# MarcoMeter/endless-memory-gym

Hardware: AMD Instinct MI355X
Metric: env steps/sec (aggregate) (higher is better)
Workload: dtype u8; 1 GPU; MortarMayhem-Grid-v0, 65536 envs/GPU x 1 GPU, 84x84x3 obs (u8_xyc), same-step auto-reset, uniform random actions generated on device; env_id=MortarMayhem-Grid-v0, envs_per_gpu=65536, envs_total=65536, parallelism=env-sharded x1, no data-path collective

## Files before the change

endless-memory-gym_amd/csrc/mg_mortar.hip:

```cpp
#include <memory>

#include "mg_atlas_v1.hpp"
#include "mg_lab.hpp"
#include "mg_option_sets.hpp"
#include "mg_stamps.hpp"
#include "mg_mortar_types.hpp"
#include "mg_mortar_compose.hpp"
#include "mg_mortar_step.hpp"
#include "mg_mortar_one_launch.hpp"

namespace mg {
using namespace v1;

__global__ __launch_bounds__(256) void mortar_init_kernel(int n, MortarState* state) {
    int i = blockIdx.x * blockDim.x + threadIdx.x;
    if (i >= n) return;
    MortarState s;
    memset(&s, 0, sizeof(s));
    s.disp_sprite = 0xFF;
    state[i] = s;
}

__global__ __launch_bounds__(256) void mortar_gt64_kernel(int n, const MortarState* state, double* out) {
    const int i = blockIdx.x * blockDim.x + threadIdx.x;
    if (i >= n) return;
    const MortarState s = state[i];
    out[2 * i] = s.tx / 5.0;
    out[2 * i + 1] = s.ty / 5.0;
}

__global__ __launch_bounds__(256) void mortar_debug_desc_kernel(MortarParams P0, int n, MortarIO io, MortarDesc* out) {
    const int i = blockIdx.x * blockDim.x + threadIdx.x;
    if (i >= n) return;
    const MortarParams& P = io.set_of ? io.sets[set_index(io.set_of, i)] : P0;
    const MortarState s = io.state[i];
    const uint8_t* cmds = io.cmds + (size_t)i * P.cmd_cap;
    MortarDesc d = io.desc[i];
    {
        const bool have = s.disp_sprite != 0xFF;
        const int cx = (have && !s.disp_is_agent) ? s.disp_x : s.ax, cy = (have && !s.disp_is_agent) ? s.disp_y : s.ay;
        d.sx = (int16_t)(cx - P.sprite_dim / 2);
        d.sy = (int16_t)(cy - P.sprite_dim / 2);
        d.sprite = have ? s.disp_sprite : (uint8_t)0;
        d.tmpl = (uint16_t)((s.tiles_on && P.visual_feedback) ? 1 + s.tx * P.N + s.ty : 0);
        d.glyph_x0 = (int16_t)P.glyph_x0;
    }
    d.glyph = 0xFF;
    if (s.vis_pos < s.vis_len) {
        const int idx = (int)s.dbg_pops, period = s.show_dur + s.show_delay;
        io.state[i].dbg_pops = s.dbg_pops + 1;
        if (idx >= 0 && idx < (int)s.vis_len && period > 0) {
            const int k = idx / period, w = idx % period;
            d.glyph = (w < s.show_dur) ? cmds[s.vis_base + k] : (uint8_t)9;
        }
    }
    const int r = P.tile / 2;
    d.ring_x = (int16_t)(P.arena_x0 + P.tile * s.tx + P.tile / 2 - r);
    d.ring_y = (int16_t)(P.arena_x0 + P.tile * s.ty + P.tile / 2 - r);
    d.ring_on = 1;
    out[i] = d;
}

static const double SCALE = 0.25;

class MortarFamily : public Family {
   public:
    MortarFamily(int variant_id, int n) : Family(n), P_(sets_[0].P) {
        memset(&P_, 0, sizeof(P_));
        const int variant = variant_id >= 3 ? variant_id - 3 : variant_id;
        P_.variant = variant;
        P_.taskb = variant_id >= 3;
        agent_scale_ = 1.0 * SCALE;
        agent_speed_ = 12.0 * SCALE;
        P_.N = variant == V_ENDLESS ? 6 : 5;
        P_.allowed = variant == V_GRID ? 5 : 9;
        P_.visual_feedback = 1;
        P_.max_steps = -1;
        P_.initial_count = 1;
        P_.cmd_cap = variant == V_ENDLESS ? 512 : 32;
        if (variant == V_ENDLESS) {
            const int cap = lab_int("MEMGYM_EMM_CMD_CAP", 0);
            if (cap >= 4 && cap <= 512) P_.cmd_cap = cap;
        }
        MortarOpt& O = sets_[0];
        O.st_command_count.set(P_.command_count, {10});
        O.st_show_dur.set(P_.show_dur, {3});
        O.st_show_delay.set(P_.show_delay, {1});
        O.st_expl_dur.set(P_.expl_dur, {variant == V_GRID ? 2 : 6});
        O.st_expl_delay.set(P_.expl_delay, {variant == V_GRID ? 6 : 18});
        P_.r_fail = 0.0;
        P_.r_succ = 0.1;
        P_.r_ep_succ = 0.0;
        P_.r_new = 0.0;
        state_.alloc(n);
        cmds_.alloc((size_t)n * P_.cmd_cap);
        desc_.alloc(n);
        tdesc_.alloc(n);
        rng_.alloc(n);
        err_.alloc();
        claims_.alloc((size_t)((n + 255) / 256) * 4);
        rescues_.alloc(1);
        sets_.alloc();
        launch(mortar_init_kernel, dim3((n + 255) / 256), dim3(256), 0, 0, n, state_.p);
        MG_HIP(hipDeviceSynchronize());
        rebuild();
        sets_.defaults = P_;
    }

    void set_capacity(const std::string& what, int64_t v) override {
        if (!(P_.variant == V_ENDLESS && what == "commands")) return Family::set_capacity(what, v);
        if (v < 4 || v > 32768) throw OptionError{-3, "commands: 4 .. 32,768"};
        if (seeded_) throw std::runtime_error("mg_set_capacity: before the first reset");
        if (2 * P_.initial_count > v) throw OptionError{-3, "commands: below twice the initial_command_count in force"};
        MG_HIP(hipDeviceSynchronize());
        P_.cmd_cap = (int)v;
        cmds_.alloc((size_t)n_ * P_.cmd_cap);
        sets_.refresh_geometry();
    }
    int64_t capacity(const std::string& what) const override {
        if (P_.variant == V_ENDLESS && what == "commands") return P_.cmd_cap;
        return Family::capacity(what);
    }
    void want_done_flag(uint32_t* flag_dev, uint32_t ticket) override {
        flag_dev_ = flag_dev;
        flag_ticket_ = ticket;
    }
    bool done_flag_stored() override {
        const bool stored = flag_stored_;
        flag_stored_ = false;
        return stored;
    }
    int action_dim() const override { return P_.variant == V_GRID ? 1 : 2; }
    int gt_dim() const override { return P_.variant == V_ENDLESS ? 2 : 0; }
    int vec_dim() const override { return P_.taskb ? VEC_DIM : 0; }
    void bind_vector_obs(float* dev) override { vec_ = dev; }
    const char* info_name(int k) const override {
        if (P_.variant == V_ENDLESS) return k == 0 ? "commands_completed" : (k == 1 ? "max_command_sequence" : nullptr);
        return k == 0 ? "success" : (k == 1 ? "commands_completed" : nullptr);
    }

    void set_option(const std::string& key, const double* v, int n) override { set_option_set(0, key, v, n); }
    void set_option_set(int set, const std::string& key, const double* v, int n) override {
        MortarOpt& O = sets_.ensure(set);
        MortarParams& P = O.P;
        const bool endless = P_.variant == V_ENDLESS;
        const OptionArg A{set, key, v, n, dirty_};
        if (key == "agent_scale") A.geometry(agent_scale_, v[0]);
        else if (key == "allowed_commands") {
            int a = A.integer();
            if (a < 4 || a > 9) throw OptionError{-4, "assert 4 <= allowed_commands <= 9"};
            P.allowed = a;
        }
        else if (!P_.taskb && key == "command_show_duration") O.st_show_dur.set(P.show_dur, A.int_list(1, 65535));
        else if (!P_.taskb && key == "command_show_delay") O.st_show_delay.set(P.show_delay, A.int_list(0, 65535));
        else if (key == "explosion_duration") O.st_expl_dur.set(P.expl_dur, A.int_list(1, 65535));
        else if (key == "explosion_delay") O.st_expl_delay.set(P.expl_delay, A.int_list(1, 65535));
        else if (key == "visual_feedback") P.visual_feedback = A.flag();
        else if (key == "reward_command_failure") P.r_fail = v[0];
        else if (key == "reward_command_success") P.r_succ = v[0];
        else if (endless && key == "max_steps") P.max_steps = A.integer();
        else if (endless && key == "initial_command_count") {
            int c = A.integer();
            if (c < 1 || c > P_.cmd_cap / 2) throw OptionError{-3, "initial_command_count out of the supported range"};
            P.initial_count = c;
        }
        else if (endless && key == "reward_new_command_success") P.r_new = v[0];
        else if (!endless && key == "arena_size") {
            int a = A.integer();
            if (a < 2 || a > 6) throw OptionError{-4, "assert 2 <= arena_size <= 6"};
            if (a != P_.N) A.geometry(P_.N, a);
        }
        else if (!endless && key == "command_count") O.st_command_count.set(P.command_count, A.int_list(1, P_.taskb ? VEC_DIM / 9 : P_.cmd_cap));
        else if (!endless && key == "reward_episode_success") P.r_ep_succ = v[0];
        else if (P_.variant != V_GRID && key == "agent_speed") A.geometry(agent_speed_, v[0]);
        else throw OptionError{-2, "unknown reset parameter " + key};
    }
    void bind_option_sets(const int32_t* set_of_dev) override { sets_.bind(set_of_dev); }

    void reset(const int64_t* seeds, const uint8_t* mask, void* obs, float* gt, hipStream_t s) override {
        if (dirty_) rebuild();
        require_seeded(seeds);
        for (size_t k = 0; k < sets_.size(); ++k) {
            const MortarOpt& O = sets_[k];
            const long long n_max = P_.variant == V_ENDLESS ? O.P.initial_count : O.st_command_count.max(O.P.command_count);
            if (!P_.taskb && n_max * ((long long)O.st_show_dur.max(O.P.show_dur) + O.st_show_delay.max(O.P.show_delay)) > 65535)
                throw OptionError{-3, "command_count x (command_show_duration + command_show_delay) exceeds the 65,535 entries of this build's display schedule"};
        }
        if (seeds) seeded_ = true;
        sets_.upload(s);
        with_bool(sets_.per_set(), [&](auto PS) {
            launch(mortar_reset_kernel<decltype(PS)::value>, dim3((n_ + 255) / 256), dim3(256), 0, s, P_, n_, io(), seeds, mask, gt_dim() ? gt : nullptr);
        });
        reset_frames(mask, [&](const uint8_t* m) { launch_raster_sparse<MortarComposer>(desc_.p, atlas_->dev(), obs, obs_format, n_, s, m); },
                     [&] { raster(obs, s); });
    }

    void step(const int32_t* actions, void* obs, float* reward, uint8_t* done, float* gt, const mg_info_buffers* info,
              int autoreset, hipStream_t s) override {
        struct Consume {
            uint32_t*& flag;
            ~Consume() { flag = nullptr; }
        } consume{flag_dev_};
        flag_stored_ = false;
        const mg_info_buffers ib = begin_step(info);
        sets_.upload(s);
        const MortarStepArgs sa{P_, n_, io(), actions, reward, done, gt_dim() ? gt : nullptr, ib, autoreset, nullptr};
        if (one_byte_format() && fuse_step() && !sets_.per_set() && !capturing(s)) {
            epoch_ = epoch_ % 255u + 1u;
            ++ticket_;
            const int logic_wgs = (n_ + 255) / 256;
            const int frames = frames_grid(n_);
            static const bool logic_last = lab_flag("MEMGYM_LAB_LOGIC_LAST", false);
            const bool store_flag = flag_dev_ && n_ == 1 && gt_dim() == 0 && obs_format == MG_OBS_U8_XYC;
            auto one_launch = [&](auto kernel, const MortarStepArgs& a, uint32_t* flag, uint32_t flag_ticket) {
                launch(kernel, dim3(logic_wgs + frames), dim3(256), RASTER_LDS, s, a, logic_wgs, logic_last ? frames : 0, epoch_, ticket_,
                               claims_.p, rescues_.p, atlas_->dev(), obs, flag, flag_ticket);
            };
            prof.begin(1, s);
            if (store_flag) {
                one_launch(mortar_step_raster_kernel<true>, sa, flag_dev_, flag_ticket_);
            } else if (ib.final_obs_dev && autoreset) {
                MortarStepArgs fa = sa;
                fa.tdesc = tdesc_.p;
                with_one_byte_format(obs_format, [&](auto F) { one_launch(mortar_step_raster_kernel<false, true, decltype(F)::value>, fa, nullptr, 0u); });
            } else {
                with_one_byte_format(obs_format, [&](auto F) { one_launch(mortar_step_raster_kernel<false, false, decltype(F)::value>, sa, nullptr, 0u); });
            }
            check_launch();
            ++one_launch_steps_;
            flag_stored_ = store_flag;
            prof.end(1, s);
            return;
        }
        prof.begin(0, s);
        const int sb = step_block(256);
        with_bool(sets_.per_set(), [&](auto PS) { launch(mortar_step_kernel<decltype(PS)::value>, dim3((n_ + sb - 1) / sb), dim3(sb), 0, s, sa); });
        end_logic(s);
        prof.begin(1, s);
        raster(obs, s);
        prof.end(1, s);
    }

    std::vector<std::pair<void*, size_t>> state_blobs() override {
        std::vector<std::pair<void*, size_t>> v = {{state_.p, state_.bytes()}, {cmds_.p, cmds_.bytes()}};
        rng_.blobs(v);
        return v;
    }

    void ground_truth64(double* out, hipStream_t s) override {
        if (!gt_dim() || !out) return;
        launch_checked(mortar_gt64_kernel, dim3((n_ + 255) / 256), dim3(256), 0, s, n_, state_.p, out);
    }
    bool debug_counter(const std::string& name, int64_t* out) override {
        if (name == "cmd_list_max" || name == "cmd_list_ge12") {
            std::vector<MortarState> h(n_);
            MG_HIP(hipDeviceSynchronize());
            MG_HIP(hipMemcpy(h.data(), state_.p, sizeof(MortarState) * (size_t)n_, hipMemcpyDeviceToHost));
            int64_t mx = 0, ge = 0;
            for (const MortarState& s : h) {
                mx = s.num_cmds > mx ? s.num_cmds : mx;
                ge += s.num_cmds >= 12;
            }
            *out = name == "cmd_list_max" ? mx : ge;
            return true;
        }
        if (name == "one_launch_steps") {
            *out = one_launch_steps_;
            return true;
        }
        if (name != "one_launch_rescues") return false;
        uint32_t v = 0;
        MG_HIP(hipMemcpy(&v, rescues_.p, sizeof v, hipMemcpyDeviceToHost));
        *out = (int64_t)v;
        return true;
    }

    void raster_debug(void* frames, hipStream_t s) override {
        debug_frames<MortarDesc>(
            s, [&](MortarDesc* dbg) { launch(mortar_debug_desc_kernel, dim3((n_ + 255) / 256), dim3(256), 0, s, P_, n_, io(), dbg); },
            [&](MortarDesc* dbg) { launch_raster<MortarDebugComposer>(dbg, atlas_->dev(), frames, MG_OBS_U8_XYC, n_, s); });
    }

   private:
    uint32_t* flag_dev_ = nullptr;
    uint32_t flag_ticket_ = 0;
    bool flag_stored_ = false;
    int64_t one_launch_steps_ = 0;
    uint32_t ticket_ = 0;
    uint32_t epoch_ = 0;
    bool one_byte_format() const { return obs_format == MG_OBS_U8_XYC || obs_format == MG_OBS_U8_CYX; }
    static bool fuse_step() {
        static const bool on = lab_flag("MEMGYM_MORTAR_FUSE", true);
        return on;
    }
    static bool capturing(hipStream_t s) {
        hipStreamCaptureStatus st = hipStreamCaptureStatusNone;
        return hipStreamIsCapturing(s, &st) == hipSuccess && st != hipStreamCaptureStatusNone;
    }
    MortarIO io() {
        MortarIO o;
        o.state = state_.p;
        o.cmds = cmds_.p;
        o.rng = rng_.view();
        o.desc = desc_.p;
        o.vec = vec_;
        o.err = err_.dev;
        o.sets = sets_.dev();
        o.set_of = sets_.set_of();
        return o;
    }

    void rebuild() {
        int radius = 0;
        std::vector<Stamp> sprites = build_agent_sprites(P_.variant == V_GRID ? 1.0 * SCALE : agent_scale_, &radius);
        std::vector<Stamp> glyphs = build_glyphs(SCALE);
        P_.tile = (int)(56 * SCALE);
        P_.arena_x0 = SCREEN / 2 - ((P_.tile * P_.N) >> 1);
        P_.radius = radius;
        P_.sprite_dim = sprites[0].w;
        double inv = 1.0 / std::sqrt(2.0);
        P_.v_axis = (1.0 / 1.0) * agent_speed_;
        P_.v_diag = inv * agent_speed_;
        P_.v_axis_i = (int)P_.v_axis;
        P_.v_diag_i = (int)P_.v_diag;
        P_.off_lo = (int)(-8 * SCALE);
        P_.off_hi = (int)(8 * SCALE);

        atlas_.reset(new Atlas());
        for (auto& sp : sprites) atlas_->add_stamp(sp);
        for (auto& g : glyphs) atlas_->add_stamp(g);
        {
            const int r = P_.tile / 2;
            Stamp ring_stamp(2 * r, 2 * r);
            circle(ring_stamp, r, r, r, (int)(8 * SCALE), 6);
            atlas_->add_stamp(ring_stamp);
        }
        atlas_->set_templates(build_mortar_templates(P_.N, SCALE, SCREEN));
        atlas_->upload();
        P_.glyph_x0 = (int)((SCREEN / 2) - std::floor(88 * SCALE / 2));
        dirty_ = false;
        sets_.refresh_geometry();
    }

    struct MortarOpt {
        MortarParams P;
        OptListStore st_command_count, st_show_dur, st_show_delay, st_expl_dur, st_expl_delay;
        static void copy_geometry(MortarParams& d, const MortarParams& s) {
            d.variant = s.variant; d.N = s.N; d.taskb = s.taskb; d.cmd_cap = s.cmd_cap; d.arena_x0 = s.arena_x0; d.tile = s.tile;
            d.radius = s.radius; d.sprite_dim = s.sprite_dim; d.glyph_x0 = s.glyph_x0; d.v_axis_i = s.v_axis_i; d.v_diag_i = s.v_diag_i;
            d.off_lo = s.off_lo; d.off_hi = s.off_hi; d.v_axis = s.v_axis; d.v_diag = s.v_diag;
        }
    };

    void raster_only(void* obs, const uint8_t* only, hipStream_t s) override {
        launch_raster<MortarComposer>(desc_.p, atlas_->dev(), obs, obs_format, n_, s, only);
        check_launch();
    }
    bool keeps_final_obs(hipStream_t s) override {
        static const bool wanted = lab_flag("MEMGYM_MORTAR_FINAL_FUSED", true);
        return wanted && one_byte_format() && fuse_step() && !sets_.per_set() && !capturing(s);
    }

    void raster(void* obs, hipStream_t s) { raster_only(obs, nullptr, s); }

    OptionSets<MortarOpt> sets_;
    MortarParams& P_;
    std::unique_ptr<Atlas> atlas_;
    double agent_scale_, agent_speed_;
    float* vec_ = nullptr;
    DevArray<MortarState> state_;
    DevArray<uint8_t> cmds_;
    DevArray<MortarDesc> desc_, tdesc_;
    DevArray<uint32_t> claims_, rescues_;
};

Family* make_mortar(int variant, int num_envs) { return new MortarFamily(variant, num_envs); }

}

#ifdef MG_LAB
extern "C" int mg_lab_set_window_offsets(const long long* off, int n) {
    long long v[16] = {0};
    for (int i = 0; i < n && i < 16; ++i) v[i] = off[i];
    return hipMemcpyToSymbol(HIP_SYMBOL(mg::v1::g_lab_win_off), v, sizeof v) == hipSuccess ? 0 : -1;
}
#endif
```

endless-memory-gym_amd/csrc/mg_mortar_one_launch.hpp:

```cpp
#pragma once
#include "mg_mortar_compose.hpp"
#include "mg_mortar_step.hpp"

namespace mg {
using namespace v1;

constexpr unsigned long long RESCUE_AFTER_TICKS = 20000;
template <bool DONE_FLAG, bool FINAL = false, int FMT = MG_OBS_U8_XYC>
__global__ __launch_bounds__(256, 7) void mortar_step_raster_kernel(MortarStepArgs a, int logic_wgs, int logic_base, uint32_t epoch,
                                                                    uint32_t ticket, uint32_t* claims, uint32_t* rescues,
                                                                    RasterAtlas A, void* __restrict__ obs, uint32_t* done_flag, uint32_t done_ticket) {
    const int n = a.n;
    const int tid = threadIdx.x, lane = tid & 63;
    const int rel = (int)blockIdx.x - logic_base;
    const bool is_logic = rel >= 0 && rel < logic_wgs;
    auto claim = [&](int q) -> bool {
        uint32_t old = 0;
        if (lane == 0) old = __hip_atomic_exchange(claims + q, ticket, __ATOMIC_RELAXED, __HIP_MEMORY_SCOPE_AGENT);
        return (uint32_t)__builtin_amdgcn_readfirstlane((int)old) != ticket;
    };
    if (is_logic) {
        const int q = rel * 4 + (tid >> 6), i = q * 64 + lane;
#if defined(MG_LABV) && MG_LABV >= 1
        if (i < n) mortar_step_body<true, false, false, FINAL>(i, a, epoch);
#else
        if (i < n) mortar_step_body<true, true, false, FINAL>(i, a, epoch, claims + q, ticket);
#endif
        return;
    }
    extern __shared__ __attribute__((aligned(16))) uint8_t smem[];
    RasterCtx R = make_ctx(smem, A);
    const int stride = (int)gridDim.x - logic_wgs;
    for (int v = (int)blockIdx.x < logic_base ? (int)blockIdx.x : (int)blockIdx.x - logic_wgs; v < n; v += stride) {
        const int env = xcd_grouped_frame(v, n);
        const uint32_t* src = reinterpret_cast<const uint32_t*>(a.io.desc + env);
        uint32_t w[4];
        bool tried = false;
        unsigned long long t0 = 0;
        for (int polls = 0;; ++polls) {
            w[3] = (uint32_t)__builtin_amdgcn_readfirstlane((int)__hip_atomic_load(src + 3, __ATOMIC_RELAXED, __HIP_MEMORY_SCOPE_AGENT));
            if ((w[3] >> 24) == epoch) break;
#if defined(MG_LABV) && MG_LABV >= 2
            if (false) {
#else
            if (polls == 0) t0 = wall_clock64();
            if (!tried && (polls & 15) == 15 && wall_clock64() - t0 >= RESCUE_AFTER_TICKS) {
#endif
                tried = true;
                if (claim(env >> 6)) {
                    const MortarStepArgs MG_KERNARG_AS* ka = kernarg_reread<MortarStepArgs>();
                    int i = (env >> 6) * 64 + lane;
                    asm volatile("" : "+v"(i));
                    if (i < n) mortar_step_body<true, false, false, FINAL>(i, *(const MortarStepArgs*)ka, epoch);
                    if (lane == 0) atomicAdd(rescues, 1u);
                    continue;
                }
            }
            __builtin_amdgcn_s_sleep(4);
        }
        asm volatile("" ::: "memory");
        w[0] = __hip_atomic_load(src + 0, __ATOMIC_RELAXED, __HIP_MEMORY_SCOPE_AGENT);
        w[1] = __hip_atomic_load(src + 1, __ATOMIC_RELAXED, __HIP_MEMORY_SCOPE_AGENT);
        w[2] = __hip_atomic_load(src + 2, __ATOMIC_RELAXED, __HIP_MEMORY_SCOPE_AGENT);
        MortarDesc d;
        memcpy(&d, w, sizeof(d));
        if constexpr (FINAL) {
            if (d.ring_on) {
                const uint32_t* tsrc = reinterpret_cast<const uint32_t*>(a.tdesc + env);
                uint32_t tw[4];
#pragma unroll
                for (int k = 0; k < 4; ++k) tw[k] = __hip_atomic_load(tsrc + k, __ATOMIC_RELAXED, __HIP_MEMORY_SCOPE_AGENT);
                MortarDesc td;
                memcpy(&td, tw, sizeof(td));
                int tt = tid;
                asm volatile("" : "+v"(tt));
                R.tid = tt;
                MortarComposer::compose(&td, R);
                __syncthreads();
                store_frame<FMT, false>(smem, a.info.final_obs_dev, env, tt);
                __syncthreads();
            }
        }
        if (MortarComposer::skip(&d)) continue;
        int t = tid;
        asm volatile("" : "+v"(t));
        R.tid = t;
        MortarComposer::compose(&d, R);
        __syncthreads();
        store_frame<FMT, false>(smem, obs, env, t);
        __syncthreads();
    }
    if constexpr (DONE_FLAG) {
        __builtin_amdgcn_fence(__ATOMIC_RELEASE, "");
        __syncthreads();
        if (tid == 0) __hip_atomic_store(done_flag, done_ticket, __ATOMIC_RELAXED, __HIP_MEMORY_SCOPE_SYSTEM);
    }
}
}
```

endless-memory-gym_amd/csrc/mg_mortar_step.hpp:

```cpp
#pragma once
#include "mg_mortar_types.hpp"

namespace mg {
constexpr uint32_t pack_deltas(const int (&v)[9]) {
    uint32_t m = 0;
    for (int c = 0; c < 9; ++c) m |= (uint32_t)(v[c] + 1) << (2 * c);
    return m;
}
constexpr int kDxHost[9] = {1, 0, -1, 0, 0, 1, 1, -1, -1}, kDyHost[9] = {0, 1, 0, -1, 0, 1, -1, 1, -1};
constexpr uint32_t CMD_DX_BITS = pack_deltas(kDxHost), CMD_DY_BITS = pack_deltas(kDyHost);
__device__ __forceinline__ int cmd_dx(int c) { return (int)((CMD_DX_BITS >> (2 * c)) & 3u) - 1; }
__device__ __forceinline__ int cmd_dy(int c) { return (int)((CMD_DY_BITS >> (2 * c)) & 3u) - 1; }

__device__ __forceinline__ int floordiv(int a, int b) {
    int q = a / b;
    return (a % b != 0 && a < 0) ? q - 1 : q;
}
__device__ __forceinline__ int mod6(int a) { return ((a % 6) + 6) % 6; }
__device__ __forceinline__ int round_haz(double v) { return v >= 0 ? (int)floor(v + 0.5) : -(int)floor(-v + 0.5); }

__constant__ int8_t kCmdOneHot[9] = {1, 4, 2, 3, 0, 5, 6, 7, 8};
constexpr int VEC_DIM = 180;

__device__ void mortar_reset(const MortarParams& P, MortarState& s, Pcg& g, uint8_t* cmds, MortarDesc& d, float* gt, float* vec) {
    if (s.disp_sprite != 0xFF && s.disp_is_agent) {
        s.disp_x = s.ax;
        s.disp_y = s.ay;
        s.disp_is_agent = 0;
    }
    int half = P.tile / 2;
    int tile_id = g.integers(0, P.N * P.N);
    int cx = P.arena_x0 + P.tile * (tile_id / P.N) + half;
    int cy = P.arena_x0 + P.tile * (tile_id % P.N) + half;
    if (P.variant == V_ENDLESS || (P.taskb && P.variant == V_FREE)) {
        cx += g.integers(P.off_lo, P.off_hi);
        cy += g.integers(P.off_lo, P.off_hi);
    }
    s.ax = (int16_t)cx;
    s.ay = (int16_t)cy;
    s.rot8 = 0;
    int nx = floordiv(cx - P.arena_x0, P.tile), ny = floordiv(cy - P.arena_x0, P.tile);
    s.nx = (int8_t)nx;
    s.ny = (int8_t)ny;
    s.gx = (uint8_t)nx;
    s.gy = (uint8_t)ny;

    int n;
    if (P.variant == V_ENDLESS) {
        n = P.initial_count;
        for (int i = 0; i < n; ++i) cmds[i] = (uint8_t)g.integers(0, P.allowed);
    } else {
        n = choice(g, P.command_count);
        int px = nx, py = ny;
        for (int i = 0; i < n; ++i) {
            uint32_t valid = 0;
#pragma unroll
            for (int c = 0; c < 9; ++c) {
                const int qx = px + cmd_dx(c), qy = py + cmd_dy(c);
                if (c < P.allowed && qx >= 0 && qx < P.N && qy >= 0 && qy < P.N) valid |= 1u << c;
            }
            const int pick = g.integers(0, __popc(valid));
            uint32_t m = valid;
            for (int k = 0; k < pick; ++k) m &= m - 1;
            const int c = __ffs(m) - 1;
            cmds[i] = (uint8_t)c;
            px += cmd_dx(c);
            py += cmd_dy(c);
        }
    }
    s.num_cmds = (uint16_t)n;
    if (P.taskb) {
        s.show_dur = s.show_delay = 0;
    } else {
        s.show_dur = (uint16_t)choice(g, P.show_dur);
        s.show_delay = (uint16_t)choice(g, P.show_delay);
    }
    s.vis_len = (uint16_t)(n * (s.show_dur + s.show_delay));
    s.vis_base = 0;
    s.vis_pos = 1;
    s.dbg_pops = 0;
    int first = cmds[0];
    uint8_t glyph = s.show_dur > 0 ? (uint8_t)first : (uint8_t)9;
    if (P.variant == V_ENDLESS) {
        s.tx = (int8_t)mod6(nx + cmd_dx(first));
        s.ty = (int8_t)mod6(ny + cmd_dy(first));
    } else {
        s.tx = (int8_t)(nx + cmd_dx(first));
        s.ty = (int8_t)(ny + cmd_dy(first));
    }
    s.cur_cmd = 0;
    s.cmd_steps = 0;
    s.verify_step = 0;
    s.total_completed = 0;
    s.tiles_on = 0;
    s.t = 0;
    s.ep_len = 0;
    s.ep_sum = 0.0;
    s.expl_dur = (uint16_t)choice(g, P.expl_dur);
    s.expl_delay = (uint16_t)choice(g, P.expl_delay);

    d.tmpl = 0;
    d.sprite = 0;
    d.sx = (int16_t)(cx - P.sprite_dim / 2);
    d.sy = (int16_t)(cy - P.sprite_dim / 2);
    d.glyph = glyph;
    if (gt) {
        gt[0] = (float)(s.tx / 5.0);
        gt[1] = (float)(s.ty / 5.0);
    }
    if (vec) {
        for (int k = 0; k < VEC_DIM; ++k) vec[k] = 0.0f;
        for (int c = 0; c < n && c < VEC_DIM / 9; ++c) vec[9 * c + kCmdOneHot[cmds[c]]] = 1.0f;
    }
}

template <bool PS>
__global__ __launch_bounds__(256) void mortar_reset_kernel(MortarParams P0, int n, MortarIO io, const int64_t* seeds,
                                                           const uint8_t* mask, float* gt) {
    int i = blockIdx.x * blockDim.x + threadIdx.x;
    if (i >= n) return;
    const MortarParams& P = PS ? io.sets[set_index(io.set_of, i)] : P0;
    MortarDesc d;
    memset(&d, 0, sizeof(d));
    d.glyph_x0 = (int16_t)P.glyph_x0;
    if (mask && !mask[i]) {
        d.tmpl = 0xFFFF;
        io.desc[i] = d;
        return;
    }
    Pcg g;
    if (seeds) g.seed((uint64_t)seeds[i]);
    else g.load(io.rng, i);
    MortarState s = io.state[i];
    mortar_reset(P, s, g, io.cmds + (size_t)i * P.cmd_cap, d, gt ? gt + 2 * i : nullptr, io.vec ? io.vec + (size_t)i * VEC_DIM : nullptr);
    io.state[i] = s;
    g.store(io.rng, i);
    io.desc[i] = d;
}

template <bool FUSED, bool CLAIM = false, bool PS = false, bool FINAL = false>
__device__ __forceinline__ void mortar_step_body(int i, const MortarStepArgs& a, uint32_t epoch, uint32_t* claim_word = nullptr,
                                                 uint32_t ticket = 0u) {
    uint32_t claimed_by = 0u;
    if constexpr (CLAIM) {
        claimed_by = ticket + 1u;
        if ((threadIdx.x & 63) == 0) claimed_by = __hip_atomic_exchange(claim_word, ticket, __ATOMIC_RELAXED, __HIP_MEMORY_SCOPE_AGENT);
    }
    const MortarIO& io = a.io;
    const MortarParams& P = PS ? io.sets[set_index(io.set_of, i)] : a.P;
    const int32_t* const actions = a.actions;
    float* const reward_out = a.reward_out;
    uint8_t* const done_out = a.done_out;
    float* const gt = a.gt;
    const mg_info_buffers& info = a.info;
    const int autoreset = a.autoreset;
    const bool one_action = P.variant == V_GRID;
    int act0 = actions[one_action ? i : 2 * i], act1 = actions[one_action ? i : 2 * i + 1];
    Pcg g;
    bool rng_loaded = !FUSED;
    if constexpr (!FUSED) g.load(io.rng, i);
    MortarState s = io.state[i];
    asm volatile("" : "+v"(act0), "+v"(act1));
    if constexpr (!FUSED) g.pin();
    if constexpr (CLAIM) {
        asm volatile("" : "+v"(claimed_by));
        if ((uint32_t)__builtin_amdgcn_readfirstlane((int)claimed_by) == ticket) return;
    }
    uint8_t* cmds = io.cmds + (size_t)i * P.cmd_cap;
    double reward = 0.0;
    bool done = false, cap = false;
    int success = 0;
    uint8_t glyph = 0xFF;
    bool rng_used = false;

    if (s.vis_pos < s.vis_len) {
        int period = s.show_dur + s.show_delay;
        int k = s.vis_pos / period, w = s.vis_pos % period;
        glyph = (w < s.show_dur) ? cmds[s.vis_base + k] : (uint8_t)9;
        s.vis_pos++;
        if (P.variant != V_ENDLESS || s.disp_sprite == 0xFF) {
            s.disp_sprite = 0;
            s.disp_is_agent = 1;
        }
    } else {
        int ax = s.ax, ay = s.ay;
        if (P.variant == V_GRID) {
            int a = act0;
            int rot = s.rot8 * 45;
            if (a == 1) rot = (rot + 90) % 360;
            if (a == 2) rot = (rot + 270) % 360;
            int gx = s.gx, gy = s.gy;
            if (a == 3) {
                int face = rot / 90;
                if (face == 0) { if (gy > 0) gy--; }
                else if (face == 3) { if (gx < P.N - 1) gx++; }
                else if (face == 2) { if (gy < P.N - 1) gy++; }
                else { if (gx > 0) gx--; }
                ax = P.arena_x0 + P.tile * gx + P.tile / 2;
                ay = P.arena_x0 + P.tile * gy + P.tile / 2;
            }
            s.gx = (uint8_t)gx;
            s.gy = (uint8_t)gy;
            s.rot8 = (uint8_t)(rot / 45);
        } else {
            int a0 = act0, a1 = act1;
            int dxs = a0 == 1 ? -1 : (a0 == 2 ? 1 : 0), dys = a1 == 1 ? -1 : (a1 == 2 ? 1 : 0);
            int rot = s.rot8 * 45;
            if (a0 == 1) rot = 90;
            if (a0 == 2) rot = 270;
            if (a1 == 1) rot = 0;
            if (a1 == 2) rot = 180;
            if (dxs < 0 && dys < 0) rot = 45;
            if (dxs < 0 && dys > 0) rot = 135;
            if (dxs > 0 && dys < 0) rot = 315;
            if (dxs > 0 && dys > 0) rot = 225;
            s.rot8 = (uint8_t)(rot / 45);
            bool diag = dxs != 0 && dys != 0;
            if (P.variant == V_FREE) {
                int v = diag ? P.v_diag_i : P.v_axis_i;
                ax += dxs * v;
                ay += dys * v;
                int lo = P.arena_x0 + P.radius, hi = P.arena_x0 + P.tile * P.N - P.radius;
                ax = ax > hi ? hi : ax;
                ax = ax < lo ? lo : ax;
                ay = ay > hi ? hi : ay;
                ay = ay < lo ? lo : ay;
            } else {
                double v = diag ? P.v_diag : P.v_axis;
                ax = round_haz((double)ax + dxs * v);
                ay = round_haz((double)ay + dys * v);
                double left = P.arena_x0, right = P.arena_x0 + P.tile * P.N, off = P.radius * 0.5;
                double x = ax, y = ay;
                if (x > right + off) x = left - off;
                if (x < left - off) x = right + off;
                if (y > right + off) y = left - off;
                if (y < left - off) y = right + off;
                ax = round_haz(x);
                ay = round_haz(y);
            }
        }
        s.ax = (int16_t)ax;
        s.ay = (int16_t)ay;
        s.disp_sprite = s.rot8;
        s.disp_is_agent = 1;
        int nx = floordiv(ax - P.arena_x0, P.tile), ny = floordiv(ay - P.arena_x0, P.tile);
        s.nx = (int8_t)nx;
        s.ny = (int8_t)ny;
        bool on_target = (nx == s.tx) && (ny == s.ty);

        bool verify = (s.cmd_steps % s.expl_delay == 0) && s.cmd_steps > 0;
        if (verify && !s.tiles_on) {
            if (s.cur_cmd < s.num_cmds) {
                s.cur_cmd++;
                s.tiles_on = 1;
                if (on_target) {
                    reward += P.r_succ;
                    if (P.variant == V_ENDLESS) {
                        s.total_completed++;
                        if (s.cur_cmd == s.num_cmds) reward += P.r_new;
                    }
                } else {
                    done = true;
                    reward += P.r_fail;
                }
            }
            if (s.cur_cmd >= s.num_cmds) {
                if (P.variant == V_ENDLESS) {
                    if (!rng_loaded) g.load(io.rng, i);
                    rng_loaded = true;
                    rng_used = true;
                    int nc = g.integers(0, P.allowed);
                    if (s.num_cmds < P.cmd_cap) {
                        cmds[s.num_cmds] = (uint8_t)nc;
                        s.vis_base = s.num_cmds;
                        s.num_cmds++;
                    } else {
                        raise_error(io.err, ERR_CMD_OVERFLOW);
                        done = true;
                        cap = true;
                        s.vis_base = (uint16_t)(s.num_cmds - 1);
                    }
                    s.cur_cmd = 0;
                    s.verify_step = 0;
                    s.vis_pos = 0;
                    s.vis_len = (uint16_t)(s.show_dur + s.show_delay);
                    s.dbg_pops = 0;
                } else {
                    done = true;
                    success = 1;
                    reward += P.r_ep_succ;
                }
            }
            s.cmd_steps = 1;
        }
        if (s.tiles_on) {
            if (s.verify_step % s.expl_dur == 0 && s.verify_step > 0) {
                s.tiles_on = 0;
                s.verify_step = 0;
                if (s.cur_cmd < s.num_cmds) {
                    int c = cmds[s.cur_cmd];
                    if (P.variant == V_ENDLESS) {
                        s.tx = (int8_t)mod6(s.tx + cmd_dx(c));
                        s.ty = (int8_t)mod6(s.ty + cmd_dy(c));
                    } else {
                        s.tx = (int8_t)(s.tx + cmd_dx(c));
                        s.ty = (int8_t)(s.ty + cmd_dy(c));
                    }
                }
            } else {
                if (!on_target) {
                    done = true;
                    reward = P.r_fail;
                }
                s.verify_step++;
            }
        } else {
            s.cmd_steps++;
        }
    }

    if (P.variant == V_ENDLESS) {
        s.t++;
        if (s.t == P.max_steps) done = true;
    }
    s.ep_sum += reward;
    s.ep_len++;

    if (done) {
        if (info.ep_reward_dev) info.ep_reward_dev[i] = s.ep_sum;
        if (info.ep_length_dev) info.ep_length_dev[i] = s.ep_len;
        if (P.variant == V_ENDLESS) {
            if (info.aux_dev[0]) info.aux_dev[0][i] = (float)s.total_completed;
            if (info.aux_dev[1]) info.aux_dev[1][i] = (float)(s.num_cmds > 1 ? s.num_cmds - 1 : 0);
        } else {
            if (info.aux_dev[0]) info.aux_dev[0][i] = (float)success;
            if (info.aux_dev[1]) info.aux_dev[1][i] = (float)((double)((int)s.cur_cmd - 1 + success) / (double)s.num_cmds);
        }
    }
    reward_out[i] = (float)reward;
    if (info.reward64_dev) info.reward64_dev[i] = reward;
    done_out[i] = done ? 1 : 0;
    if (info.capacity_dev) info.capacity_dev[i] = cap ? 1 : 0;

    MortarDesc d;
    memset(&d, 0, sizeof(d));
    d.glyph_x0 = (int16_t)P.glyph_x0;
    if (done && autoreset) {
        if constexpr (FINAL) {
            MortarDesc td;
            memset(&td, 0, sizeof(td));
            td.glyph_x0 = (int16_t)P.glyph_x0;
            const int tcx = s.disp_is_agent ? s.ax : s.disp_x, tcy = s.disp_is_agent ? s.ay : s.disp_y;
            td.sx = (int16_t)(tcx - P.sprite_dim / 2);
            td.sy = (int16_t)(tcy - P.sprite_dim / 2);
            td.sprite = s.disp_sprite;
            td.glyph = glyph;
            td.tmpl = (uint16_t)((s.tiles_on && P.visual_feedback) ? 1 + s.tx * P.N + s.ty : 0);
            uint32_t tw[4];
            memcpy(tw, &td, sizeof(tw));
            uint32_t* tdst = reinterpret_cast<uint32_t*>(&a.tdesc[i]);
            __hip_atomic_store(tdst + 0, tw[0], __ATOMIC_RELAXED, __HIP_MEMORY_SCOPE_AGENT);
            __hip_atomic_store(tdst + 1, tw[1], __ATOMIC_RELAXED, __HIP_MEMORY_SCOPE_AGENT);
            __hip_atomic_store(tdst + 2, tw[2], __ATOMIC_RELAXED, __HIP_MEMORY_SCOPE_AGENT);
            __hip_atomic_store(tdst + 3, tw[3], __ATOMIC_RELAXED, __HIP_MEMORY_SCOPE_AGENT);
        }
        if (!rng_loaded) g.load(io.rng, i);
        rng_loaded = true;
        rng_used = true;
        mortar_reset(P, s, g, cmds, d, (gt && P.variant == V_ENDLESS) ? gt + 2 * i : nullptr, io.vec ? io.vec + (size_t)i * VEC_DIM : nullptr);
        if constexpr (FINAL) d.ring_on = 1;
    } else {
        int cx = s.disp_is_agent ? s.ax : s.disp_x, cy = s.disp_is_agent ? s.ay : s.disp_y;
        d.sx = (int16_t)(cx - P.sprite_dim / 2);
        d.sy = (int16_t)(cy - P.sprite_dim / 2);
        d.sprite = s.disp_sprite;
        d.glyph = glyph;
        d.tmpl = (uint16_t)((s.tiles_on && P.visual_feedback) ? 1 + s.tx * P.N + s.ty : 0);
        if (gt && P.variant == V_ENDLESS) {
            gt[2 * i] = (float)(s.tx / 5.0);
            gt[2 * i + 1] = (float)(s.ty / 5.0);
        }
    }
    if (rng_used) g.store(io.rng, i);
    io.state[i] = s;
    if constexpr (FUSED) {
        d.epoch = (uint8_t)epoch;
        uint32_t w[4];
        memcpy(w, &d, sizeof(w));
        uint32_t* dst = reinterpret_cast<uint32_t*>(&io.desc[i]);
        __hip_atomic_store(dst + 0, w[0], __ATOMIC_RELAXED, __HIP_MEMORY_SCOPE_AGENT);
        __hip_atomic_store(dst + 1, w[1], __ATOMIC_RELAXED, __HIP_MEMORY_SCOPE_AGENT);
        __hip_atomic_store(dst + 2, w[2], __ATOMIC_RELAXED, __HIP_MEMORY_SCOPE_AGENT);
        asm volatile("s_waitcnt vmcnt(0)" ::: "memory");
        __hip_atomic_store(dst + 3, w[3], __ATOMIC_RELAXED, __HIP_MEMORY_SCOPE_AGENT);
    } else {
        io.desc[i] = d;
    }
}

template <bool PS>
__global__ __launch_bounds__(256) void mortar_step_kernel(MortarStepArgs a) {
    const int i = blockIdx.x * blockDim.x + threadIdx.x;
    if (i < a.n) mortar_step_body<false, false, PS>(i, a, 0u);
}
}
```

endless-memory-gym_amd/csrc/mg_mortar_types.hpp:

```cpp
#pragma once
#include "mg_family.hpp"
#include "mg_raster_v1.hpp"

namespace mg {
using namespace v1;
enum { V_GRID = 0, V_FREE = 1, V_ENDLESS = 2 };

struct MortarParams {
    int variant, N, allowed, visual_feedback, max_steps, initial_count;
    int taskb;
    int cmd_cap;
    int arena_x0, tile;
    int radius, sprite_dim;
    int glyph_x0;
    int v_axis_i, v_diag_i;
    int off_lo, off_hi;
    double v_axis, v_diag;
    OptList command_count, show_dur, show_delay, expl_dur, expl_delay;
    double r_fail, r_succ, r_ep_succ, r_new;
};

struct __attribute__((aligned(16))) MortarState {
    int16_t ax, ay;
    int16_t disp_x, disp_y;
    uint8_t rot8 : 3;
    uint8_t disp_is_agent : 1;
    uint8_t tiles_on : 1;
    uint8_t disp_sprite;
    int8_t tx, ty;
    int8_t nx, ny;
    uint16_t num_cmds, cur_cmd;
    uint16_t vis_pos, vis_len, vis_base;
    uint16_t cmd_steps, verify_step;
    uint16_t show_dur, show_delay, expl_dur, expl_delay;
    uint8_t gx, gy;
    int32_t ep_len, t, total_completed;
    uint32_t dbg_pops;
    double ep_sum;
};
static_assert(sizeof(MortarState) == 64, "MortarState must be 64 bytes");

struct __attribute__((aligned(16))) MortarDesc {
    int16_t sx, sy;
    uint16_t tmpl;
    uint8_t sprite;
    uint8_t glyph;
    int16_t glyph_x0;
    int16_t ring_x, ring_y;
    uint8_t ring_on;
    uint8_t epoch;
};
static_assert(sizeof(MortarDesc) == 16, "MortarDesc must be 16 bytes");
constexpr int STAMP_SPRITE0 = 0, STAMP_GLYPH0 = 8, STAMP_RING = 18;

struct MortarIO {
    MortarState* state;
    uint8_t* cmds;
    RngSoA rng;
    MortarDesc* desc;
    float* vec;
    int* err;
    const MortarParams* sets;
    const int32_t* set_of;
};
constexpr int ERR_CMD_OVERFLOW = 32;

struct MortarStepArgs {
    MortarParams P;
    int n;
    MortarIO io;
    const int32_t* actions;
    float* reward_out;
    uint8_t* done_out;
    float* gt;
    mg_info_buffers info;
    int autoreset;
    MortarDesc* tdesc;
};
}
```

Before: 291.3 million env steps/s.

## Pack logic-to-raster descriptor handover into a single 64-bit atomic word

The fused step kernel's logic waves now publish each env's render descriptor as one packed 64-bit word (with the epoch in the top byte) into a separate handover array, instead of four 32-bit atomic stores to the 16-byte MortarDesc with a waitcnt before the epoch word. Raster waves poll that single 64-bit word and unpack it, so they no longer need three follow-up loads, and the unconditional s_waitcnt on the logic side is dropped except in the final-obs or ordered paths. The terminal descriptor is packed the same way. The cost is fewer bits per field (15-bit template, 4-bit sprite and glyph), plus an extra handover array and a plain desc store that stay live.

```diff
diff --git a/endless-memory-gym_amd/csrc/mg_mortar.hip b/endless-memory-gym_amd/csrc/mg_mortar.hip
--- a/endless-memory-gym_amd/csrc/mg_mortar.hip
+++ b/endless-memory-gym_amd/csrc/mg_mortar.hip
@@ -99,6 +99,7 @@
         rng_.alloc(n);
         err_.alloc();
         claims_.alloc((size_t)((n + 255) / 256) * 4);
+        handover_.alloc(n);
         rescues_.alloc(1);
         sets_.alloc();
         launch(mortar_init_kernel, dim3((n + 255) / 256), dim3(256), 0, 0, n, state_.p);
@@ -167,7 +168,7 @@
         else if (endless && key == "reward_new_command_success") P.r_new = v[0];
         else if (!endless && key == "arena_size") {
             int a = A.integer();
-            if (a < 2 || a > 6) throw OptionError{-4, "assert 2 <= arena_size <= 6"};
+            if (a < 2 || a > MORTAR_MAX_N) throw OptionError{-4, "assert 2 <= arena_size <= 6"};
             if (a != P_.N) A.geometry(P_.N, a);
         }
         else if (!endless && key == "command_count") O.st_command_count.set(P.command_count, A.int_list(1, P_.taskb ? VEC_DIM / 9 : P_.cmd_cap));
@@ -204,7 +205,7 @@
         flag_stored_ = false;
         const mg_info_buffers ib = begin_step(info);
         sets_.upload(s);
-        const MortarStepArgs sa{P_, n_, io(), actions, reward, done, gt_dim() ? gt : nullptr, ib, autoreset, nullptr};
+        const MortarStepArgs sa{P_, n_, io(), actions, reward, done, gt_dim() ? gt : nullptr, ib, autoreset, handover_.p, nullptr};
         if (one_byte_format() && fuse_step() && !sets_.per_set() && !capturing(s)) {
             epoch_ = epoch_ % 255u + 1u;
             ++ticket_;
@@ -370,8 +371,9 @@
     float* vec_ = nullptr;
     DevArray<MortarState> state_;
     DevArray<uint8_t> cmds_;
-    DevArray<MortarDesc> desc_, tdesc_;
+    DevArray<MortarDesc> desc_;
     DevArray<uint32_t> claims_, rescues_;
+    DevArray<uint64_t> handover_, tdesc_;
 };
 
 Family* make_mortar(int variant, int num_envs) { return new MortarFamily(variant, num_envs); }
diff --git a/endless-memory-gym_amd/csrc/mg_mortar_handover.hpp b/endless-memory-gym_amd/csrc/mg_mortar_handover.hpp
--- /dev/null
+++ b/endless-memory-gym_amd/csrc/mg_mortar_handover.hpp
@@ -0,0 +1,43 @@
+#pragma once
+#include <cstdint>
+
+namespace mg {
+constexpr int HANDOVER_SX_SHIFT = 0, HANDOVER_SY_SHIFT = 16, HANDOVER_TMPL_SHIFT = 32, HANDOVER_RING_SHIFT = 47, HANDOVER_SPRITE_SHIFT = 48,
+              HANDOVER_GLYPH_SHIFT = 52, HANDOVER_EPOCH_SHIFT = 56;
+constexpr uint32_t HANDOVER_TMPL_NONE = 0x7FFF;
+constexpr uint32_t HANDOVER_TMPL_MAX = 0x7FFE;
+constexpr uint32_t HANDOVER_NIBBLE_NONE = 0xF;
+static_assert(HANDOVER_SX_SHIFT == 0 && HANDOVER_SY_SHIFT - HANDOVER_SX_SHIFT == 16 && HANDOVER_TMPL_SHIFT - HANDOVER_SY_SHIFT == 16, "sx, sy: 16 bits each");
+static_assert(HANDOVER_RING_SHIFT - HANDOVER_TMPL_SHIFT == 15 && HANDOVER_SPRITE_SHIFT - HANDOVER_RING_SHIFT == 1, "tmpl 15 bits, ring_on 1");
+static_assert(HANDOVER_GLYPH_SHIFT - HANDOVER_SPRITE_SHIFT == 4 && HANDOVER_EPOCH_SHIFT - HANDOVER_GLYPH_SHIFT == 4, "sprite, glyph: 4 bits each");
+static_assert(HANDOVER_EPOCH_SHIFT + 8 == 64 && HANDOVER_EPOCH_SHIFT - 32 == 24, "the epoch is the top byte of the word (and of its high dword)");
+
+struct Handover {
+    int32_t sx, sy;
+    uint32_t tmpl, ring_on, sprite, glyph, epoch;
+};
+
+constexpr uint32_t handover_lo(int32_t sx, int32_t sy) { return ((uint32_t)sx & 0xFFFFu) | ((uint32_t)sy & 0xFFFFu) << (HANDOVER_SY_SHIFT - HANDOVER_SX_SHIFT); }
+constexpr uint32_t handover_hi(uint32_t tmpl, uint32_t ring_on, uint32_t sprite, uint32_t glyph, uint32_t epoch) {
+    return (tmpl == 0xFFFFu ? HANDOVER_TMPL_NONE : tmpl & 0x7FFFu) << (HANDOVER_TMPL_SHIFT - 32) | (ring_on ? 1u : 0u) << (HANDOVER_RING_SHIFT - 32) |
+           (sprite == 0xFFu ? HANDOVER_NIBBLE_NONE : sprite & 0xFu) << (HANDOVER_SPRITE_SHIFT - 32) |
+           (glyph == 0xFFu ? HANDOVER_NIBBLE_NONE : glyph & 0xFu) << (HANDOVER_GLYPH_SHIFT - 32) | (epoch & 0xFFu) << (HANDOVER_EPOCH_SHIFT - 32);
+}
+constexpr uint64_t pack_handover(int32_t sx, int32_t sy, uint32_t tmpl, uint32_t ring_on, uint32_t sprite, uint32_t glyph, uint32_t epoch) {
+    return (uint64_t)handover_hi(tmpl, ring_on, sprite, glyph, epoch) << 32 | handover_lo(sx, sy);
+}
+constexpr Handover unpack_handover(uint32_t lo, uint32_t hi) {
+    const uint32_t tmpl = hi & 0x7FFFu, sprite = (hi >> (HANDOVER_SPRITE_SHIFT - 32)) & 0xFu, glyph = (hi >> (HANDOVER_GLYPH_SHIFT - 32)) & 0xFu;
+    return Handover{(int32_t)(int16_t)(uint16_t)(lo & 0xFFFFu), (int32_t)(int16_t)(uint16_t)(lo >> 16), tmpl == HANDOVER_TMPL_NONE ? 0xFFFFu : tmpl,
+                    (hi >> (HANDOVER_RING_SHIFT - 32)) & 1u, sprite == HANDOVER_NIBBLE_NONE ? 0xFFu : sprite, glyph == HANDOVER_NIBBLE_NONE ? 0xFFu : glyph,
+                    hi >> (HANDOVER_EPOCH_SHIFT - 32)};
+}
+constexpr Handover unpack_handover(uint64_t w) { return unpack_handover((uint32_t)w, (uint32_t)(w >> 32)); }
+
+static_assert(unpack_handover(pack_handover(-1, -32768, 36, 1, 7, 9, 255)).sx == -1 && unpack_handover(pack_handover(-1, -32768, 36, 1, 7, 9, 255)).sy == -32768,
+              "sx, sy are sign-extended");
+static_assert(unpack_handover(pack_handover(0, 0, 0xFFFF, 0, 0xFF, 0xFF, 1)).tmpl == 0xFFFF && unpack_handover(pack_handover(0, 0, 0xFFFF, 0, 0xFF, 0xFF, 1)).sprite == 0xFF &&
+                  unpack_handover(pack_handover(0, 0, 0xFFFF, 0, 0xFF, 0xFF, 1)).glyph == 0xFF,
+              "the none codes come back as MortarDesc's");
+static_assert(pack_handover(0, 0, 0, 0, 0, 0, 0) == 0, "a zeroed word is epoch 0: never a one-launch epoch");
+}
diff --git a/endless-memory-gym_amd/csrc/mg_mortar_one_launch.hpp b/endless-memory-gym_amd/csrc/mg_mortar_one_launch.hpp
--- a/endless-memory-gym_amd/csrc/mg_mortar_one_launch.hpp
+++ b/endless-memory-gym_amd/csrc/mg_mortar_one_launch.hpp
@@ -6,6 +6,14 @@
 using namespace v1;
 
 constexpr unsigned long long RESCUE_AFTER_TICKS = 20000;
+__device__ __forceinline__ MortarDesc desc_from_handover(uint32_t lo, uint32_t hi, int glyph_x0) {
+    const Handover f = unpack_handover(lo, hi);
+    MortarDesc d;
+    d.sx = (int16_t)f.sx, d.sy = (int16_t)f.sy, d.tmpl = (uint16_t)f.tmpl, d.sprite = (uint8_t)f.sprite, d.glyph = (uint8_t)f.glyph;
+    d.glyph_x0 = (int16_t)glyph_x0;
+    d.ring_x = d.ring_y = 0, d.ring_on = (uint8_t)f.ring_on, d.reserved = 0;
+    return d;
+}
 template <bool DONE_FLAG, bool FINAL = false, int FMT = MG_OBS_U8_XYC>
 __global__ __launch_bounds__(256, 7) void mortar_step_raster_kernel(MortarStepArgs a, int logic_wgs, int logic_base, uint32_t epoch,
                                                                     uint32_t ticket, uint32_t* claims, uint32_t* rescues,
@@ -22,9 +30,9 @@
     if (is_logic) {
         const int q = rel * 4 + (tid >> 6), i = q * 64 + lane;
 #if defined(MG_LABV) && MG_LABV >= 1
-        if (i < n) mortar_step_body<true, false, false, FINAL>(i, a, epoch);
+        if (i < n) mortar_step_body<true, false, false, FINAL, DONE_FLAG>(i, a, epoch);
 #else
-        if (i < n) mortar_step_body<true, true, false, FINAL>(i, a, epoch, claims + q, ticket);
+        if (i < n) mortar_step_body<true, true, false, FINAL, DONE_FLAG>(i, a, epoch, claims + q, ticket);
 #endif
         return;
     }
@@ -33,13 +41,15 @@
     const int stride = (int)gridDim.x - logic_wgs;
     for (int v = (int)blockIdx.x < logic_base ? (int)blockIdx.x : (int)blockIdx.x - logic_wgs; v < n; v += stride) {
         const int env = xcd_grouped_frame(v, n);
-        const uint32_t* src = reinterpret_cast<const uint32_t*>(a.io.desc + env);
-        uint32_t w[4];
+        const uint64_t* src = a.handover + env;
+        uint32_t lo, hi;
         bool tried = false;
         unsigned long long t0 = 0;
         for (int polls = 0;; ++polls) {
-            w[3] = (uint32_t)__builtin_amdgcn_readfirstlane((int)__hip_atomic_load(src + 3, __ATOMIC_RELAXED, __HIP_MEMORY_SCOPE_AGENT));
-            if ((w[3] >> 24) == epoch) break;
+            const uint64_t w = __hip_atomic_load(src, __ATOMIC_RELAXED, __HIP_MEMORY_SCOPE_AGENT);
+            lo = (uint32_t)__builtin_amdgcn_readfirstlane((int)(uint32_t)w);
+            hi = (uint32_t)__builtin_amdgcn_readfirstlane((int)(uint32_t)(w >> 32));
+            if ((hi >> (HANDOVER_EPOCH_SHIFT - 32)) == epoch) break;
 #if defined(MG_LABV) && MG_LABV >= 2
             if (false) {
 #else
@@ -51,33 +61,25 @@
                     const MortarStepArgs MG_KERNARG_AS* ka = kernarg_reread<MortarStepArgs>();
                     int i = (env >> 6) * 64 + lane;
                     asm volatile("" : "+v"(i));
-                    if (i < n) mortar_step_body<true, false, false, FINAL>(i, *(const MortarStepArgs*)ka, epoch);
+                    if (i < n) mortar_step_body<true, false, false, FINAL, DONE_FLAG>(i, *(const MortarStepArgs*)ka, epoch);
                     if (lane == 0) atomicAdd(rescues, 1u);
                     continue;
                 }
             }
             __builtin_amdgcn_s_sleep(4);
         }
-        asm volatile("" ::: "memory");
-        w[0] = __hip_atomic_load(src + 0, __ATOMIC_RELAXED, __HIP_MEMORY_SCOPE_AGENT);
-        w[1] = __hip_atomic_load(src + 1, __ATOMIC_RELAXED, __HIP_MEMORY_SCOPE_AGENT);
-        w[2] = __hip_atomic_load(src + 2, __ATOMIC_RELAXED, __HIP_MEMORY_SCOPE_AGENT);
-        MortarDesc d;
-        memcpy(&d, w, sizeof(d));
+        const MortarDesc d = desc_from_handover(lo, hi, a.P.glyph_x0);
         if constexpr (FINAL) {
             if (d.ring_on) {
-                const uint32_t* tsrc = reinterpret_cast<const uint32_t*>(a.tdesc + env);
-                uint32_t tw[4];
-#pragma unroll
-                for (int k = 0; k < 4; ++k) tw[k] = __hip_atomic_load(tsrc + k, __ATOMIC_RELAXED, __HIP_MEMORY_SCOPE_AGENT);
-                MortarDesc td;
-                memcpy(&td, tw, sizeof(td));
+                const MortarStepArgs MG_KERNARG_AS* ka = kernarg_reread<MortarStepArgs>();
+                const uint64_t tw = __hip_atomic_load(ka->tdesc + env, __ATOMIC_RELAXED, __HIP_MEMORY_SCOPE_AGENT);
+                const MortarDesc td = desc_from_handover((uint32_t)__builtin_amdgcn_readfirstlane((int)(uint32_t)tw), (uint32_t)__builtin_amdgcn_readfirstlane((int)(uint32_t)(tw >> 32)), a.P.glyph_x0);
                 int tt = tid;
                 asm volatile("" : "+v"(tt));
                 R.tid = tt;
                 MortarComposer::compose(&td, R);
                 __syncthreads();
-                store_frame<FMT, false>(smem, a.info.final_obs_dev, env, tt);
+                store_frame<FMT, false>(smem, ka->info.final_obs_dev, env, tt);
                 __syncthreads();
             }
         }
diff --git a/endless-memory-gym_amd/csrc/mg_mortar_step.hpp b/endless-memory-gym_amd/csrc/mg_mortar_step.hpp
--- a/endless-memory-gym_amd/csrc/mg_mortar_step.hpp
+++ b/endless-memory-gym_amd/csrc/mg_mortar_step.hpp
@@ -138,7 +138,7 @@
     io.desc[i] = d;
 }
 
-template <bool FUSED, bool CLAIM = false, bool PS = false, bool FINAL = false>
+template <bool FUSED, bool CLAIM = false, bool PS = false, bool FINAL = false, bool ORDERED = false>
 __device__ __forceinline__ void mortar_step_body(int i, const MortarStepArgs& a, uint32_t epoch, uint32_t* claim_word = nullptr,
                                                  uint32_t ticket = 0u) {
     uint32_t claimed_by = 0u;
@@ -347,22 +347,10 @@
     d.glyph_x0 = (int16_t)P.glyph_x0;
     if (done && autoreset) {
         if constexpr (FINAL) {
-            MortarDesc td;
-            memset(&td, 0, sizeof(td));
-            td.glyph_x0 = (int16_t)P.glyph_x0;
             const int tcx = s.disp_is_agent ? s.ax : s.disp_x, tcy = s.disp_is_agent ? s.ay : s.disp_y;
-            td.sx = (int16_t)(tcx - P.sprite_dim / 2);
-            td.sy = (int16_t)(tcy - P.sprite_dim / 2);
-            td.sprite = s.disp_sprite;
-            td.glyph = glyph;
-            td.tmpl = (uint16_t)((s.tiles_on && P.visual_feedback) ? 1 + s.tx * P.N + s.ty : 0);
-            uint32_t tw[4];
-            memcpy(tw, &td, sizeof(tw));
-            uint32_t* tdst = reinterpret_cast<uint32_t*>(&a.tdesc[i]);
-            __hip_atomic_store(tdst + 0, tw[0], __ATOMIC_RELAXED, __HIP_MEMORY_SCOPE_AGENT);
-            __hip_atomic_store(tdst + 1, tw[1], __ATOMIC_RELAXED, __HIP_MEMORY_SCOPE_AGENT);
-            __hip_atomic_store(tdst + 2, tw[2], __ATOMIC_RELAXED, __HIP_MEMORY_SCOPE_AGENT);
-            __hip_atomic_store(tdst + 3, tw[3], __ATOMIC_RELAXED, __HIP_MEMORY_SCOPE_AGENT);
+            const uint64_t tw = pack_handover(tcx - P.sprite_dim / 2, tcy - P.sprite_dim / 2, (s.tiles_on && P.visual_feedback) ? 1 + s.tx * P.N + s.ty : 0,
+                                              0, s.disp_sprite, glyph, 0);
+            __hip_atomic_store(a.tdesc + i, tw, __ATOMIC_RELAXED, __HIP_MEMORY_SCOPE_AGENT);
         }
         if (!rng_loaded) g.load(io.rng, i);
         rng_loaded = true;
@@ -381,21 +369,13 @@
             gt[2 * i + 1] = (float)(s.ty / 5.0);
         }
     }
+    if constexpr (FUSED) {
+        if constexpr (FINAL || ORDERED) asm volatile("s_waitcnt vmcnt(0)" ::: "memory");
+        __hip_atomic_store(a.handover + i, pack_handover(d.sx, d.sy, d.tmpl, d.ring_on, d.sprite, d.glyph, epoch), __ATOMIC_RELAXED, __HIP_MEMORY_SCOPE_AGENT);
+    }
     if (rng_used) g.store(io.rng, i);
     io.state[i] = s;
-    if constexpr (FUSED) {
-        d.epoch = (uint8_t)epoch;
-        uint32_t w[4];
-        memcpy(w, &d, sizeof(w));
-        uint32_t* dst = reinterpret_cast<uint32_t*>(&io.desc[i]);
-        __hip_atomic_store(dst + 0, w[0], __ATOMIC_RELAXED, __HIP_MEMORY_SCOPE_AGENT);
-        __hip_atomic_store(dst + 1, w[1], __ATOMIC_RELAXED, __HIP_MEMORY_SCOPE_AGENT);
-        __hip_atomic_store(dst + 2, w[2], __ATOMIC_RELAXED, __HIP_MEMORY_SCOPE_AGENT);
-        asm volatile("s_waitcnt vmcnt(0)" ::: "memory");
-        __hip_atomic_store(dst + 3, w[3], __ATOMIC_RELAXED, __HIP_MEMORY_SCOPE_AGENT);
-    } else {
-        io.desc[i] = d;
-    }
+    io.desc[i] = d;
 }
 
 template <bool PS>
diff --git a/endless-memory-gym_amd/csrc/mg_mortar_types.hpp b/endless-memory-gym_amd/csrc/mg_mortar_types.hpp
--- a/endless-memory-gym_amd/csrc/mg_mortar_types.hpp
+++ b/endless-memory-gym_amd/csrc/mg_mortar_types.hpp
@@ -1,5 +1,6 @@
 #pragma once
 #include "mg_family.hpp"
+#include "mg_mortar_handover.hpp"
 #include "mg_raster_v1.hpp"
 
 namespace mg {
@@ -48,7 +49,7 @@
     int16_t glyph_x0;
     int16_t ring_x, ring_y;
     uint8_t ring_on;
-    uint8_t epoch;
+    uint8_t reserved;
 };
 static_assert(sizeof(MortarDesc) == 16, "MortarDesc must be 16 bytes");
 constexpr int STAMP_SPRITE0 = 0, STAMP_GLYPH0 = 8, STAMP_RING = 18;
@@ -75,6 +76,9 @@
     float* gt;
     mg_info_buffers info;
     int autoreset;
-    MortarDesc* tdesc;
+    uint64_t* handover;
+    uint64_t* tdesc;
 };
+constexpr int MORTAR_MAX_N = 6;
+static_assert(MORTAR_MAX_N * MORTAR_MAX_N <= (int)HANDOVER_TMPL_MAX, "a template index the host accepts does not fit the hand-over word");
 }
```

After: 300.3 million env steps/s (median of 6 runs). 3.1% higher.
